# grospy/bitcoincashplus

Measured on AMD Instinct MI355X. Metric: equihash_200_9_solutions_per_sec, higher is better.
Workload: dtype uint32; 1 GPU; model=Equihash(200,9) mainnet PoW solver (BLAKE2b, K=9 collision rounds), global_batch=96, seq_len=2097152, parallelism=dp1 (nonce-space), solvers_in_flight=2, full=False, verified_solutions=0, gpu_cpu_verifier_disagreements=0, rows_dropped_all_nonces=231992, pairs_dropped_all_nonces=346543, candidates_dropped_all_nonces=0

## Files before the change

### csrc/kernels/equihash_solver.hip

```cpp
#include <hip/hip_runtime.h>

#include "crypto/hashes.h"
#include "kernels/blake2b_device.h"
#include "kernels/equihash_pow.h"
#include "kernels/gpu_api.h"
#include "kernels/hip_util.h"

#include <algorithm>
#include <cstdlib>
#include <cstring>
#include <stdexcept>
#include <utility>

#ifndef BCP_EH_XCD_MAP
#define BCP_EH_XCD_MAP 1
#endif
#ifndef BCP_EH_PF_SLICES
#define BCP_EH_PF_SLICES 3
#endif
#ifndef BCP_EH_GEN_HPT
#define BCP_EH_GEN_HPT 2
#endif
#ifndef BCP_EH_GEN_NT
#define BCP_EH_GEN_NT 512
#endif
#ifndef BCP_EH_PRUNE_FROM
#define BCP_EH_PRUNE_FROM 9
#endif
#ifndef BCP_EH_MP_LATE
#define BCP_EH_MP_LATE 1
#endif
#ifndef BCP_EH_MP_LATE_FROM
#define BCP_EH_MP_LATE_FROM 8
#endif
#ifndef BCP_EH_GW
#define BCP_EH_GW 4
#endif
#ifndef BCP_EH_GROUPS_DEFAULT
#define BCP_EH_GROUPS_DEFAULT(batch) ((batch) >= 48 ? (batch) / 24 : 1)
#endif

namespace bcpk {

template <int N_, int K_, int BB_, int CAP_, int NT_, int GENWG_, int NTG_, int MAXCAND_, int CAP4_ = CAP_,
          int CAP3_ = CAP_, int WGCU_ = 1, int GNT_ = 512, int GHPT_ = 2, int CAPF_ = 0, int MPX_ = 0, int GW_ = 0>
struct EhCfg {
    static constexpr int N = N_, K = K_;
    static constexpr int DB = N / (K + 1);
    static constexpr int BB = BB_;
    static constexpr int RB = DB - BB_;
    static constexpr int NB = 1 << BB_;
    static constexpr int NRESTS = 1 << RB;
    static constexpr int CAP = CAP_;
    static constexpr int CAPF = CAPF_ > 0 ? CAPF_ : CAP3_;
    static constexpr int MPX = MPX_;
    static constexpr int cap(int round) {
        return round == K_ ? CAPF : words(round - 1) >= 5 ? CAP_ : words(round - 1) == 4 ? CAP4_ : CAP3_;
    }
    static constexpr int AREA_NF = CAP_ > CAP4_ ? (CAP_ > CAP3_ ? CAP_ : CAP3_) : (CAP4_ > CAP3_ ? CAP4_ : CAP3_);
    static constexpr int AREA = AREA_NF > CAPF ? AREA_NF : CAPF;
    static constexpr int NT = NT_;
    static constexpr int NW = NT_ / 64;
    static constexpr int GW = GW_;
    static constexpr int RNT = NT_ - 64 * GW_;
    static constexpr int WGCU = WGCU_;
    static constexpr int LDS_BUDGET = 160 * 1024 / WGCU_;
    static constexpr int INIT = 1 << (DB + 1);
    static constexpr int GENWG = GENWG_;
    static constexpr int NTG = NTG_;
    static constexpr int GNT = GNT_, GHPT = GHPT_;
    static constexpr int RPW = INIT / GENWG_;
    static constexpr int IPH = 512 / N;
    static constexpr int NBYTES = N / 8;
    static constexpr int MAXCAND = MAXCAND_;
    static constexpr int L = 1 << K;
    static constexpr int bits(int stage) { return N - stage * DB - BB_; }
    static constexpr int words(int stage) { return (bits(stage) + 31) / 32; }
    static constexpr int WMAX = words(0);
    static constexpr int IB = AREA <= 4096 ? 12 : 13;
    static constexpr int DH = 16 - IB;
    static constexpr uint32_t DHM = (1u << DH) - 1;
    static constexpr int DX = 2 * DH;
    static constexpr int DR = BB_ > DX ? BB_ - DX : 0;
    static constexpr uint32_t RMASK = (1u << DR) - 1;
    static constexpr uint32_t IMASK = ((1u << IB) - 1) * 0x10001u;
    static constexpr bool cp(int stage) {
        return stage >= 1 && stage < K && 32 * words(stage) - bits(stage) >= DR;
    }
    static constexpr uint32_t rmask(int stage) { return cp(stage) ? RMASK : 0u; }
    static constexpr int sw(int stage) { return stage == 0 ? words(0) : words(stage) + (cp(stage) ? 1 : 2); }
    static constexpr size_t ROWS = (size_t)NB * AREA;
    static constexpr bool H16 = NB > 512;
    static constexpr int HW = H16 ? NB / 2 : NB;
    static_assert(RPW * GENWG_ == INIT && RPW < 65535, "generation split");
    static_assert(RB > 0 && DB < 32, "digit geometry");
    static_assert(AREA < (1 << IB), "LDS row indices in parent words and signatures");
    static_assert(NT_ % 64 == 0 && NT_ <= 1024 && (NB <= NT_ || NB % NT_ == 0) && NB <= NTG_ && NT_ / 64 <= 64,
                  "workgroup shape");
    static_assert(words(K - 1) == 1, "final round keeps whole rows in one LDS word");
    static_assert(GW_ == 0 || (WGCU_ == 1 && RNT >= 128 && (NB <= RNT || NB % RNT == 0)), "carrying workgroup shape");
};

#ifndef BCP_EH_CAPF
#define BCP_EH_CAPF 6016
#endif
using Cfg200_9 = EhCfg<200, 9, 9, 4416, 1024, 512, 1024, 256, 4864, 5120, 1, BCP_EH_GEN_NT, BCP_EH_GEN_HPT, BCP_EH_CAPF, 0, BCP_EH_GW>;
using Cfg96_5 = EhCfg<96, 5, 7, 1280, 256, 256, 256, 256, 1280, 1280, 1, 512, 2, 0, 1, 1>;
using Cfg48_5 = EhCfg<48, 5, 3, 512, 64, 8, 64, 256>;

constexpr uint32_t NIL = 0xffffffffu;
constexpr uint32_t OOB = 0x80000000u;
typedef uint32_t u2v __attribute__((ext_vector_type(2)));
typedef uint32_t u3v __attribute__((ext_vector_type(3)));
typedef uint32_t u4v __attribute__((ext_vector_type(4)));

template <int CTRL, int ROWMASK = 0xf>
__device__ __forceinline__ uint32_t dpp0(uint32_t x) {
    return (uint32_t)__builtin_amdgcn_update_dpp(0, (int)x, CTRL, ROWMASK, 0xf, false);
}
template <bool MAX> __device__ __forceinline__ uint32_t wave_incl(uint32_t x) {
    auto op = [](uint32_t a, uint32_t b) -> uint32_t { return MAX ? (a > b ? a : b) : a + b; };
    x = op(x, dpp0<0x111>(x));
    x = op(x, dpp0<0x112>(x));
// ... 296 lines not shown
    for (int q = 0; q < G::RPT; ++q) {
        const uint32_t d = rk[q] & 0xffff;
        const uint32_t pos = base[d] + (rk[q] >> 16);
        const uint32_t slot = d * C::AREA + pos;
        const bool ok = pos < OCAP;
        const uint32_t g = g0 + (q / C::IPH) * NTG + tid;
        const uint32_t li = g * C::IPH + (q % C::IPH);
        row_store<W0>(rs, ok ? slot * (SW0 * 4) : OOB, rw[q]);
        __builtin_amdgcn_raw_buffer_store_b32(li, rl, ok ? slot * 4 : OOB, 0, 0);
    }
    }
}

__device__ __forceinline__ uint64_t pack_tri(uint32_t d, uint32_t i, uint32_t j) {
    return ((uint64_t)d << 32) | (j << 16) | i;
}
template <class C> __host__ __device__ __forceinline__ uint32_t cpack(uint32_t d, uint32_t i, uint32_t j) {
    return i | (j << 16) | ((d & C::DHM) << C::IB) | (((d >> C::DH) & C::DHM) << (16 + C::IB));
}
template <class C> __host__ __device__ __forceinline__ uint32_t cunpack_d(uint32_t pw, uint32_t lastword) {
    return ((pw >> C::IB) & C::DHM) | (((pw >> (16 + C::IB)) & C::DHM) << C::DH) | ((lastword & C::RMASK) << C::DX);
}

#define EH_STAMP(k)                                                                                  \
    do {                                                                                             \
        if constexpr (STAMP) {                                                                       \
            if (threadIdx.x == 0) stamps[(size_t)bk * 16 + (k)] = __builtin_amdgcn_s_memtime();        \
        }                                                                                            \
    } while (0)

template <class C> constexpr int un_walk_bend(int cap) { return (cap * 2 + 3) / 4 * 4; }
template <class C> constexpr int un_walk_list(int cap) { return un_walk_bend<C>(cap) + C::NRESTS * 4; }
template <class C> constexpr int round_nt(int stage, bool carry) { return carry && stage < C::K ? C::RNT : C::NT; }
template <class C> constexpr int round_mp(int stage, bool carry = false) {
    const int nt = round_nt<C>(stage, carry);
    return stage == C::K ? 1
                         : (C::AREA_NF + nt - 1) / nt + C::MPX +
                               (C::K == 9 && stage >= BCP_EH_MP_LATE_FROM ? BCP_EH_MP_LATE : 0);
}
template <class C> constexpr int round_un(int stage, bool carry = false) {
    const int cap = C::cap(stage);
    if (stage == C::K) return un_walk_list<C>(cap);
    const int pairs = round_mp<C>(stage, carry) * round_nt<C>(stage, carry) * 4;
    const int walk = un_walk_list<C>(cap) + pairs;
    return walk > pairs ? walk : pairs;
}
template <class C> constexpr int round_lds(int stage, bool prune, bool carry = false) {
    const int WR = C::words(stage - 1);
    const int WI = WR;
    const int cap = C::cap(stage);
    const int pruneb = prune ? cap * 4 + (C::cp(stage - 1) ? 0 : (cap * 2 + 3) / 4 * 4) : 0;
    const int hists = stage == C::K ? 12 : 2 * C::HW * 4 + (C::NB * (C::H16 ? 2 : 4) + 3) / 4 * 4;
    const int gen = carry ? 2 * C::NB * 4 + 16 * 8 : 0;
    return (cap * WI + 3) / 4 * 16 + pruneb + 4 + round_un<C>(stage, carry) + hists +
           (round_nt<C>(stage, carry) / 64 + 1) * 4 + gen;
}
template <class C> constexpr bool round_prunes(int stage, bool carry = false) {
    constexpr int from = C::K == 9 ? BCP_EH_PRUNE_FROM : 2;
    return (stage >= from || stage == C::K) && stage >= 2 && round_lds<C>(stage, true, carry) <= C::LDS_BUDGET;
}

template <class C> struct GenCarry {
    static constexpr int GT = C::GW > 0 ? 64 * C::GW : 64;
    static constexpr int NHASH = (C::INIT + C::IPH - 1) / C::IPH;
    static constexpr int ITERS = (C::K - 1) * C::NB;
    static constexpr int HB = ((NHASH + ITERS - 1) / ITERS + GT - 1) / GT;
    static constexpr int CH = HB * GT;
    static constexpr int RPT = HB * C::IPH;
    static constexpr int BPT = (C::NB + GT - 1) / GT;
    static_assert((long long)CH * ITERS >= NHASH, "the carrying rounds cover every hash");
};
struct EhCarry {
    const EhBaseState* states;
    uint32_t* R0;
    uint32_t* LEAF;
    uint32_t* CTR0;
    int nonces;
};

constexpr int EH_NBAR = 10;
constexpr int EH_SCAN_BARS = 2;
template <int K> __device__ __forceinline__ void eh_bar() {
    static_assert(K >= 1 && K <= EH_NBAR, "barrier outside the bucket iteration's count");
    __syncthreads();
}
#define EH_BAR_SCAN(k) static_assert((k) >= 1 && (k) + EH_SCAN_BARS - 1 <= EH_NBAR, "scan barriers")

template <class C, int STAGE>
__device__ __forceinline__ void eh_carry_gen(const EhCarry& cy, int nbk, uint32_t* ghist, uint32_t* gbase, uint64_t* gr0p) {
    using GC = GenCarry<C>;
// ... 112 lines not shown
        if (act) {
#pragma unroll
            for (int k = 0; k < GC::BPT; ++k) {
                const int b = gtid + k * GT;
                if (b < C::NB) gbase[b] = myb[k];
            }
        }
        eh_bar<9>();
        if (act) {
            const auto rs = buf_rsrc(cy.R0 + (size_t)nonce * C::ROWS * SW0, (uint32_t)(C::ROWS * SW0 * 4));
            const auto rl = buf_rsrc(cy.LEAF + (size_t)nonce * C::ROWS, (uint32_t)(C::ROWS * 4));
#pragma unroll
            for (int q = 0; q < GC::RPT; ++q) {
                const uint32_t d = rk[q] & 0xffff;
                const uint32_t pos = gbase[d < (uint32_t)C::NB ? d : 0] + (rk[q] >> 16);
                const uint32_t slot = d * C::AREA + pos;
                const bool ok = rk[q] != NIL && pos < OCAP;
                const uint32_t li = (g0 + (q / C::IPH) * GT) * C::IPH + (q % C::IPH);
                row_store<W0>(rs, ok ? slot * (SW0 * 4) : OOB, rw[q]);
                __builtin_amdgcn_raw_buffer_store_b32(li, rl, ok ? slot * 4 : OOB, 0, 0);
            }
        }
        if (more) start(bn);
        eh_bar<EH_NBAR>();
        if (!more) break;
        bk = bn;
        ++it;
    }
}

template <class C, int STAGE, bool STAMP, bool CARRY = false>
__global__ __launch_bounds__(C::NT) __attribute__((amdgpu_waves_per_eu(C::WGCU * C::NT / 256)))
void eh_round(const uint32_t* __restrict__ Rin, const uint32_t* __restrict__ CTRin, uint32_t* __restrict__ Rout,
              uint32_t* __restrict__ CTRout, uint32_t* __restrict__ ncand, uint64_t* __restrict__ cand,
              uint64_t* __restrict__ stamps, uint32_t* __restrict__ pdrop, int nbk, EhCarry carry) {
    constexpr int WI = C::words(STAGE - 1);
    constexpr int WO = (STAGE < C::K) ? C::words(STAGE) : 1;
    constexpr int CAP = C::cap(STAGE);
    constexpr bool FINAL = STAGE == C::K;
    constexpr int PDW = 2 * C::K + 2;
    static_assert(!CARRY || (C::GW > 0 && !FINAL && !STAMP), "only plain collision rounds carry generation");
    constexpr bool PRUNE = round_prunes<C>(STAGE, CARRY);
    static_assert(PRUNE == round_prunes<C>(STAGE), "a carrying round prunes like the plain one");
    static_assert(round_lds<C>(STAGE, PRUNE, CARRY) <= 160 * 1024 / C::WGCU, "round LDS budget");
    constexpr int NT = round_nt<C>(STAGE, CARRY);
    static_assert(!CARRY || NT / 64 > 1, "block_exscan runs its two barriers only with more than one wave");
    constexpr int RPL = (CAP + NT - 1) / NT;
    constexpr int MP = round_mp<C>(STAGE, CARRY);
    constexpr int SWI = C::sw(STAGE - 1);
    constexpr int SWO = STAGE < C::K ? C::sw(STAGE) : 1;
    constexpr bool CPI = C::cp(STAGE - 1);
    constexpr uint32_t RMI = C::rmask(STAGE - 1);
    constexpr int SLI = (RPL + BCP_EH_PF_SLICES - 1) / BCP_EH_PF_SLICES;
    constexpr int BPT = (C::NB + NT - 1) / NT;
    constexpr bool FOLD = !FINAL;
    using HT = std::conditional_t<C::H16, uint16_t, uint32_t>;
    __shared__ __attribute__((aligned(16))) uint32_t rows[(CAP * WI + 3) / 4 * 4];
    __shared__ uint32_t psig[PRUNE ? CAP : 1];
    __shared__ uint16_t pdw[PRUNE && !CPI ? CAP : 1];
    __shared__ uint32_t npairs;
    __shared__ __attribute__((aligned(16))) uint8_t un[round_un<C>(STAGE, CARRY)];
    static_assert(FINAL || (sizeof(un) >= (size_t)un_walk_list<C>(CAP) + (size_t)MP * NT * 4),
                  "the union holds sidx, bend and this round's MP * NT pairs");
    __shared__ uint32_t hist_[FINAL ? 1 : C::HW], cur_[FINAL ? 1 : C::HW];
    __shared__ HT base[FINAL ? 1 : C::NB];
    __shared__ uint32_t wsum[NT / 64 + 1];
    __shared__ uint32_t ghist[CARRY ? C::NB : 1], gbase[CARRY ? C::NB : 1];
    __shared__ uint64_t gr0p[CARRY ? 16 : 1];
    uint16_t* sidx = reinterpret_cast<uint16_t*>(un);
    uint32_t* bend = reinterpret_cast<uint32_t*>(un + un_walk_bend<C>(CAP));
    uint32_t* plist = reinterpret_cast<uint32_t*>(un + un_walk_list<C>(CAP));
    uint32_t* spair = FOLD ? plist : reinterpret_cast<uint32_t*>(un);
    const int tid = threadIdx.x;
    const int G = gridDim.x;
    int it = 0;
    int bk = xcd_bucket<C::NB>(blockIdx.x, 0, G, nbk);
    if (bk < 0) return;
    if constexpr (CARRY) {
        if (__builtin_amdgcn_readfirstlane(tid >> 6) >= NT / 64) {
            eh_carry_gen<C, STAGE>(carry, nbk, ghist, gbase, gr0p);
            return;
        }
    }
// ... 42 lines not shown
        dest = (x0 >> (32 - C::DB)) & (C::NB - 1);
        return keep;
    };

    auto opaque_tid = [&]() -> uint32_t {
        uint32_t t;
        asm volatile("v_mov_b32 %0, %1" : "=v"(t) : "v"(tid));
        return t;
    };
    constexpr int LWI = PRUNE ? (CPI ? WI + 1 : WI + 2) : WI;
    uint32_t nr[RPL][LWI];
    uint32_t krank[FOLD ? RPL : 1];
    int pf_bk = bk;
    uint32_t pf_n = 0;
    auto issue = [&](int u0, int u1) {
        const int nonce = pf_bk / C::NB, d = pf_bk % C::NB;
        const auto rs = buf_rsrc(Rin + ((size_t)nonce * C::ROWS + (size_t)d * C::AREA) * SWI, CAP * SWI * 4);
        const uint32_t ot = opaque_tid();
#pragma unroll
        for (int u = 0; u < RPL; ++u) {
            if (u < u0 || u >= u1) continue;
            const uint32_t r = ot + u * NT;
            row_load<LWI>(rs, r < pf_n ? r * (SWI * 4) : OOB, nr[u]);
        }
    };

    uint32_t fill = CTRin[bk];
    uint32_t n = min(fill, (uint32_t)CAP);
    pf_n = n;
    issue(0, RPL);
    if constexpr (!FINAL) {
        const auto rs_out = buf_rsrc(Rout, 0);
        const uint32_t z[SWO] = {};
#pragma unroll
        for (int u = 0; u < MP; ++u) row_store<SWO>(rs_out, OOB + 256 * u, z);
    }
    if constexpr (FOLD) {
        for (int k = tid; k < C::NRESTS; k += NT) bend[k] = 0;
        __syncthreads();
    }
    const int bk1 = xcd_bucket<C::NB>(blockIdx.x, 1, G, nbk);
    uint32_t fill_next = bk1 >= 0 ? CTRin[bk1] : 0u;
    const auto ctr_rs = buf_rsrc(CTRin, (uint32_t)nbk * 4);
    auto fill_of = [&](int b) -> uint32_t {
        return __builtin_amdgcn_raw_buffer_load_b32(ctr_rs, b >= 0 ? (uint32_t)b * 4 : OOB, 0, 0);
    };

    for (;;) {
        const int nonce = bk / C::NB, d = bk % C::NB;
        EH_STAMP(0);
        if (tid == 0 && fill > (uint32_t)CAP) atomicAdd(&pdrop[nonce * PDW + C::K + STAGE], fill - CAP);
        {
            const uint32_t ot = opaque_tid();
#pragma unroll
            for (int u = 0; u < RPL; ++u) {
                const uint32_t r = ot + u * NT;
                if (r < n) {
                    if constexpr (WI % 2 == 0) {
#pragma unroll
                        for (int w = 0; w < WI; w += 2)
                            *reinterpret_cast<u2v*>(&rows[r * WI + w]) = u2v{nr[u][w], nr[u][w + 1]};
                    } else {
#pragma unroll
                        for (int w = 0; w < WI; ++w) rows[r * WI + w] = nr[u][w];
                    }
                    if constexpr (PRUNE) {
                        psig[r] = nr[u][WI];
                        if constexpr (!CPI) pdw[r] = (uint16_t)nr[u][WI + 1];
// ... 103 lines not shown
                    uint32_t dest;
                    if (pair_keep(i, j, dest)) {
                        pv[u] = (j << 16) | i;
                        pd[u] = dest;
                        hinc(hist_, pd[u]);
                    }
                }
            }
            for (int k = tid; k < C::NRESTS; k += NT) bend[k] = 0;
            eh_bar<6>();
            EH_STAMP(4);
            uint32_t myb[BPT];
#pragma unroll
            for (int k = 0; k < BPT; ++k) {
                const int b = tid * BPT + k;
                myb[k] = 0;
                if (b < C::NB) myb[k] = atomicAdd(&CTRout[(size_t)nonce * C::NB + b], hget(hist_, b));
            }
            issue(2 * SLI, RPL);
            uint32_t start = 0;
            uint32_t np;
            EH_BAR_SCAN(7);
            if constexpr (C::H16)
                np = block_exscan<NT, BPT, uint16_t, uint16_t>(reinterpret_cast<const uint16_t*>(hist_),
                                                               reinterpret_cast<uint16_t*>(cur_), C::NB, wsum, &start);
            else
                np = block_exscan<NT, BPT>(hist_, cur_, C::NB, wsum, &start);
#pragma unroll
            for (int u = 0; u < MP; ++u)
                if (pv[u] != NIL) spair[hinc(cur_, pd[u])] = pv[u];
#pragma unroll
            for (int k = 0; k < BPT; ++k) {
                const int b = tid * BPT + k;
                if (b < C::NB) {
                    base[b] = (HT)(myb[k] - start);
                    start += hget(hist_, b);
                }
            }
            eh_bar<9>();
            EH_STAMP(5);
            constexpr uint32_t OCAP = C::cap(STAGE + 1 <= C::K ? STAGE + 1 : C::K);
            constexpr uint32_t RMO = C::rmask(STAGE);
            const auto rs_out = buf_rsrc(Rout + (size_t)nonce * C::ROWS * SWO, (uint32_t)(C::ROWS * SWO * 4));
#pragma unroll
            for (int u = 0; u < MP; ++u) {
                const uint32_t t = tid + u * NT;
                const uint32_t pr = t < np ? spair[t] : 0u;
                const uint32_t i = pr & 0xffff, j = pr >> 16;
                uint32_t x[WI + 1], o[WO];
                lds_row_xor<WI>(rows, i, j, x);
                x[WI - 1] &= ~RMI;
                x[WI] = 0;
                const uint32_t b = (x[0] >> (32 - C::DB)) & (C::NB - 1);
                const uint32_t pos = (HT)(base[b] + t);
                const bool ok = t < np && pos < OCAP;
                const uint32_t slot = b * C::AREA + pos;
#pragma unroll
                for (int w = 0; w < WO; ++w) o[w] = (x[w] << C::DB) | (x[w + 1] >> (32 - C::DB));
                uint32_t ov[SWO] = {};
#pragma unroll
                for (int w = 0; w < WO; ++w) ov[w] = o[w];
                if constexpr (C::cp(STAGE)) {
                    ov[WO - 1] |= (d >> C::DX) & RMO;
                    ov[WO] = cpack<C>(d, i, j);
                } else {
                    ov[WO] = (j << 16) | i;
                    ov[WO + 1] = d;
                }
                row_store<SWO>(rs_out, ok ? slot * (SWO * 4) : OOB, ov);
            }
        }
        eh_bar<EH_NBAR>();
        EH_STAMP(6);
        if (!more) break;
        bk = bn;
        ++it;
        fill = fn;
        n = nn;
    }
}


struct EhStages {
    const uint32_t* r[16];
};
template <class C>
__global__ __launch_bounds__(C::L < 64 ? 64 : C::L) void eh_expand(const uint32_t* __restrict__ LEAF, EhStages st,
                                                                  const uint32_t* __restrict__ ncand,
                                                                  const uint64_t* __restrict__ cand,
                                                                  uint32_t* __restrict__ out_idx,
                                                                  uint32_t* __restrict__ out_valid,
                                                                  uint32_t* __restrict__ nout,
                                                                  uint32_t* __restrict__ out_list) {
    constexpr int L = C::L;
    __shared__ uint32_t buf[2][L];
    __shared__ uint64_t tri[L / 2 > 0 ? L / 2 : 1];
    __shared__ uint32_t dup;
    const uint32_t c = blockIdx.x % C::MAXCAND;
    const uint32_t nonce = blockIdx.x / C::MAXCAND;
    const uint32_t t = threadIdx.x;
    const uint32_t nc = min(ncand[nonce], (uint32_t)C::MAXCAND);
    if (c >= nc) return;
    if (t == 0) {
        tri[0] = cand[(size_t)nonce * C::MAXCAND + c];
        dup = 0;
    }
    int cur = 0;
    for (int s = C::K; s >= 1; --s) {
        __syncthreads();
        const uint32_t cnt = 1u << (C::K - s);
        if (t < 2 * cnt) {
            const uint64_t tr = tri[t >> 1];
            const uint32_t dd = (uint32_t)(tr >> 32);
            const uint32_t r = (t & 1) ? (((uint32_t)tr >> 16) & 0xffff) : ((uint32_t)tr & 0xffff);
            const bool in = dd < (uint32_t)C::NB && r < (uint32_t)C::AREA;
            if (!in) dup = 1;
            buf[cur][t] = in ? dd * C::AREA + r : 0u;
        }
        __syncthreads();
        if (s > 1 && t < 2 * cnt) {
            const uint32_t* q = st.r[s - 1] + ((size_t)nonce * C::ROWS + buf[cur][t]) * C::sw(s - 1) + C::words(s - 1);
            if (C::cp(s - 1))
                tri[t] = ((uint64_t)cunpack_d<C>(q[0], q[-1]) << 32) | (q[0] & C::IMASK);
            else
                tri[t] = ((uint64_t)q[1] << 32) | q[0];
        }
    }
    __syncthreads();
    if (t < (uint32_t)L) buf[cur][t] = LEAF[(size_t)nonce * C::ROWS + buf[cur][t]];
    for (int l = 0; l < C::K; ++l) {
        __syncthreads();
        if (t < (uint32_t)L) {
            const uint32_t w = 1u << l;
            const uint32_t j = t & ~(2 * w - 1);
            const bool swap = buf[cur][j + w] < buf[cur][j];
            const uint32_t pos = t - j;
            const uint32_t np = swap ? (pos < w ? pos + w : pos - w) : pos;
            buf[cur ^ 1][j + np] = buf[cur][t];
        }
        cur ^= 1;
    }
    __syncthreads();
    if (t < (uint32_t)L) out_idx[((size_t)nonce * C::MAXCAND + c) * L + t] = buf[cur][t];
    const int o = cur ^ 1;
    if (t < (uint32_t)L) buf[o][t] = buf[cur][t];
    for (uint32_t k = 2; k <= (uint32_t)L; k <<= 1) {
        for (uint32_t jj = k >> 1; jj > 0; jj >>= 1) {
            __syncthreads();
            if (t < (uint32_t)L) {
                const uint32_t ixj = t ^ jj;
                if (ixj > t) {
                    const uint32_t a = buf[o][t], bb = buf[o][ixj];
                    const bool up = (t & k) == 0;
                    if ((a > bb) == up) {
                        buf[o][t] = bb;
// ... 30 lines not shown
    CBlake2b st = st_in;
    Blake2bState& s = st.MutableState();
    if (s.buflen == 128) {
        s.t[0] += 128;
        if (s.t[0] < 128) s.t[1]++;
        CBlake2b::Compress(s.h, s.buf, s.t[0], s.t[1], false);
        s.buflen = 0;
    }
    if (s.buflen + 4 > 128) throw std::runtime_error("MakeEhBaseState: g would straddle a block boundary");
    if (s.t[1] != 0) throw std::runtime_error("MakeEhBaseState: input too long");
    EhBaseState bs;
    memset(&bs, 0, sizeof(bs));
    memcpy(bs.h, s.h, sizeof(bs.h));
    unsigned char block[128] = {0};
    memcpy(block, s.buf, s.buflen);
    for (int i = 0; i < 16; ++i) memcpy(&bs.m[i], block + 8 * i, 8);
    bs.t0 = s.t[0] + s.buflen + 4;
    bs.g_byte = s.buflen;
    bs.outlen = s.outlen;
    return bs;
}

struct EquihashGpuSolver::Impl {
    unsigned n, k;
    int batch, device;
    hipStream_t stream = nullptr;
    hipEvent_t ev0 = nullptr, ev1 = nullptr;
    hipEvent_t ev_gen = nullptr, ev_rounds = nullptr;
    const Impl* after = nullptr;
    DevBuf<bcpk::EhBaseState> d_states;
    DevBuf<uint32_t> d_ctr, d_leaf, d_ncand, d_idx, d_valid, d_pdrop, d_nout, d_out;
    DevBuf<uint64_t> d_cand;
    DevBuf<uint32_t> d_rst[16];
    HostBuf<bcpk::EhBaseState> h_states;
    HostBuf<uint32_t> h_ncand, h_idx, h_ctr0, h_ctr_all, h_pdrop, h_nout, h_out;
    size_t outq = 0;
    size_t rows = 0, L = 0, maxcand = 0, nb = 0, kstages = 0;
    std::vector<size_t> caps;
    std::vector<size_t> slot_words, row_words;
    uint32_t cp_ib = 0, cp_dh = 0, cp_dhm = 0, cp_dx = 0, cp_rmask = 0, cp_imask = 0;
    std::vector<bool> compact;
    int inflight = 0;
    DevBuf<uint32_t> d_in140, d_powctr, d_win;
    HostBuf<uint32_t> h_powctr, h_win;
    size_t winw = 0;
    const bcpk::EhPowParams* pow = nullptr;
    bool pow_inflight = false;
    bool pow_collect = false;
    EhPowJob pow_job;
    int ncu = 1;
    int groups = 1;
    bool debug = false, stamp_mode = false;
    DevBuf<uint64_t> d_stamps;
    EhGpuStats stats;
    size_t bytes = 0;

    template <class C> void alloc() {
        rows = C::ROWS;
        L = C::L;
        maxcand = C::MAXCAND;
        nb = C::NB;
        caps.clear();
        for (int r = 1; r <= C::K; ++r) caps.push_back(C::cap(r));
        slot_words.clear();
        compact.clear();
        row_words.clear();
        for (int st = 0; st < C::K; ++st) {
            slot_words.push_back(C::sw(st));
            compact.push_back(C::cp(st));
            row_words.push_back(C::words(st));
        }
        kstages = C::K;
        d_states.alloc(batch);
        h_states.alloc(batch);
        static_assert(C::K <= 16, "stage arrays");
        for (int s = 0; s < C::K; ++s) d_rst[s].alloc((size_t)batch * C::ROWS * C::sw(s));
        d_ctr.alloc((size_t)C::K * batch * C::NB);
        d_leaf.alloc((size_t)batch * C::ROWS);
        cp_ib = C::IB, cp_dh = C::DH, cp_dhm = C::DHM, cp_dx = C::DX, cp_rmask = C::RMASK, cp_imask = C::IMASK;
        d_ncand.alloc(batch);
        d_pdrop.alloc((size_t)batch * (2 * C::K + 2));
        h_pdrop.alloc((size_t)batch * (2 * C::K + 2));
        d_cand.alloc((size_t)batch * C::MAXCAND);
        d_idx.alloc((size_t)batch * C::MAXCAND * C::L);
        d_valid.alloc((size_t)batch * C::MAXCAND);
        h_ncand.alloc(batch);
        d_nout.alloc(1);
        h_nout.alloc(1);
        d_out.alloc((size_t)batch * C::MAXCAND * (C::L + 2));
        h_out.alloc((size_t)batch * C::MAXCAND * (C::L + 2));
        outq = std::min<size_t>((size_t)batch * 4 + 16, (size_t)batch * C::MAXCAND);
        h_idx.alloc((size_t)C::MAXCAND * C::L);
        h_ctr0.alloc((size_t)C::K * C::NB);
        h_ctr_all.alloc((size_t)C::K * batch * C::NB);
        d_stamps.alloc((size_t)C::K * batch * C::NB * 16);
        bytes = d_leaf.n * 4 + d_ctr.n * 4 + d_idx.n * 4;
        for (int s = 0; s < C::K; ++s) bytes += d_rst[s].n * 4;
    }

    template <class C, int S, bool ST, bool CY> int round_grid(int nbk) {
        static int per_cu = -1;
        if (per_cu < 0) {
            int occ = 0;
            BCP_HIP_CHECK(hipOccupancyMaxActiveBlocksPerMultiprocessor(&occ, bcpk::eh_round<C, S, ST, CY>, C::NT, 0));
            per_cu = std::max(occ, 1);
        }
        return std::min(nbk, ncu * per_cu);
    }
    template <class C, int S> void launch_round(int noff, int gn, int next) {
        const size_t o = (size_t)noff;
        constexpr size_t PDW = 2 * C::K + 2;
        const uint32_t* rin = d_rst[S - 1].p + o * C::ROWS * C::sw(S - 1);
        uint32_t* rout = S < C::K ? d_rst[S].p + o * C::ROWS * C::sw(S < C::K ? S : 0) : nullptr;
        const uint32_t* cin = d_ctr.p + ((size_t)(S - 1) * batch + o) * C::NB;
        uint32_t* cout = S < C::K ? d_ctr.p + ((size_t)S * batch + o) * C::NB : nullptr;
        uint32_t* nc = d_ncand.p + o;
        uint64_t* cd = d_cand.p + o * C::MAXCAND;
        const int nbk = C::NB * gn;
        bcpk::EhCarry cy{};
        if constexpr (C::GW > 0 && S < C::K) {
            if (next > 0 && !stamp_mode) {
                const size_t p = o + (size_t)gn;
                cy.states = d_states.p + p;
                cy.R0 = d_rst[0].p + p * C::ROWS * C::sw(0);
                cy.LEAF = d_leaf.p + p * C::ROWS;
                cy.CTR0 = d_ctr.p + p * C::NB;
                cy.nonces = next;
                hipLaunchKernelGGL((bcpk::eh_round<C, S, false, true>), dim3(round_grid<C, S, false, true>(nbk)),
                                   dim3(C::NT), 0, stream, rin, cin, rout, cout, nc, cd, nullptr,
                                   d_pdrop.p + o * PDW, nbk, cy);
                ++stats.carry_launches;
                return;
            }
        }
        if (stamp_mode) {
            uint64_t* st = d_stamps.p + ((size_t)(S - 1) * batch + o) * C::NB * 16;
            hipLaunchKernelGGL((bcpk::eh_round<C, S, true>), dim3(round_grid<C, S, true, false>(nbk)), dim3(C::NT), 0,
                               stream, rin, cin, rout, cout, nc, cd, st, d_pdrop.p + o * PDW, nbk, cy);
        } else {
            hipLaunchKernelGGL((bcpk::eh_round<C, S, false>), dim3(round_grid<C, S, false, false>(nbk)), dim3(C::NT), 0,
                               stream, rin, cin, rout, cout, nc, cd, nullptr, d_pdrop.p + o * PDW, nbk, cy);
        }
    }
    template <class C, int... S> void launch_rounds(int noff, int gn, int next, std::integer_sequence<int, S...>) {
        (launch_round<C, S + 1>(noff, gn, next), ...);
    }

    template <class C> void alloc_pow() {
        using P = bcpk::PowCfg<C::N, C::K>;
        if (d_win.n) return;
        winw = P::WINW;
        d_in140.alloc((size_t)batch * 35);
        d_powctr.alloc(2);
        h_powctr.alloc(2);
        d_win.alloc((size_t)batch * C::MAXCAND * P::WINW);
        h_win.alloc((size_t)batch * C::MAXCAND * P::WINW);
    }

    template <class C> void launch(size_t nstates) {
        if (pow) {
            BCP_HIP_CHECK(hipMemsetAsync(d_powctr.p, 0, 2 * sizeof(uint32_t), stream));
            hipLaunchKernelGGL((bcpk::eh_nonce_states<bcpk::PowCfg<C::N, C::K>>), dim3(((int)nstates + 63) / 64), dim3(64),
                               0, stream, *pow, (int)nstates, d_in140.p, d_states.p);
        } else
            BCP_HIP_CHECK(hipMemcpyAsync(d_states.p, h_states.p, nstates * sizeof(bcpk::EhBaseState),
                                         hipMemcpyHostToDevice, stream));
        BCP_HIP_CHECK(hipMemsetAsync(d_ncand.p, 0, batch * sizeof(uint32_t), stream));
        BCP_HIP_CHECK(hipMemsetAsync(d_nout.p, 0, sizeof(uint32_t), stream));
        BCP_HIP_CHECK(hipMemsetAsync(d_pdrop.p, 0, d_pdrop.n * sizeof(uint32_t), stream));
        BCP_HIP_CHECK(hipMemsetAsync(d_ctr.p, 0, d_ctr.n * sizeof(uint32_t), stream));
        if (debug) {
            if (d_leaf.n) BCP_HIP_CHECK(hipMemsetAsync(d_leaf.p, 0xff, d_leaf.n * sizeof(uint32_t), stream));
            for (int s = 0; s < C::K; ++s)
                if (d_rst[s].n) BCP_HIP_CHECK(hipMemsetAsync(d_rst[s].p, 0xff, d_rst[s].n * sizeof(uint32_t), stream));
        }
        BCP_HIP_CHECK(hipEventRecord(ev0, stream));
        bool hdr = true;
        for (size_t i = 0; i < nstates && !pow; ++i) {
            const bcpk::EhBaseState& st = h_states.p[i];
            hdr &= st.g_byte == 12;
            for (int w = 2; w < 16; ++w) hdr &= st.m[w] == 0;
        }
        int gsz = (int)nstates;
        if (C::GW > 0 && hdr && !stamp_mode && groups > 1) {
            gsz = ((int)nstates + groups - 1) / groups;
            if (gsz >= bcpk::NXCD) gsz = (gsz + bcpk::NXCD - 1) / bcpk::NXCD * bcpk::NXCD;
        }
        const int gen_n = std::min(gsz, (int)nstates);
        uint32_t* r0 = d_rst[0].p;
        hipStream_t gs = stream;
        if (after) BCP_HIP_CHECK(hipStreamWaitEvent(gs, after->ev_gen, 0));
        constexpr bool reg = bcpk::GenReg<C, C::GNT, C::GHPT>::OK;
        if constexpr (reg) {
            using GR = bcpk::GenReg<C, C::GNT, C::GHPT>;
            const int items = GR::GWG * gen_n;
            const int grid = items;
            if (hdr)
                hipLaunchKernelGGL((bcpk::eh_gen_reg<C, true, C::GNT, C::GHPT>), dim3(grid), dim3(C::GNT), 0, gs,
                                   d_states.p, r0, d_leaf.p, d_ctr.p, items);
            else
                hipLaunchKernelGGL((bcpk::eh_gen_reg<C, false, C::GNT, C::GHPT>), dim3(grid), dim3(C::GNT), 0, gs,
                                   d_states.p, r0, d_leaf.p, d_ctr.p, items);
        } else if (hdr)
            hipLaunchKernelGGL((bcpk::eh_gen<C, true>), dim3(C::GENWG * gen_n), dim3(C::NTG), 0, gs,
                               d_states.p, r0, d_leaf.p, d_ctr.p);
        else
            hipLaunchKernelGGL((bcpk::eh_gen<C, false>), dim3(C::GENWG * gen_n), dim3(C::NTG), 0, gs,
                               d_states.p, r0, d_leaf.p, d_ctr.p);
        BCP_HIP_CHECK(hipEventRecord(ev_gen, gs));
        if (after) BCP_HIP_CHECK(hipStreamWaitEvent(stream, after->ev_rounds, 0));
        for (int noff = 0; noff < (int)nstates; noff += gsz) {
            const int gn = std::min(gsz, (int)nstates - noff);
            const int next = std::max(0, std::min(gsz, (int)nstates - noff - gsz));
            launch_rounds<C>(noff, gn, next, std::make_integer_sequence<int, C::K>{});
        }
        constexpr int EB = C::L < 64 ? 64 : C::L;
        bcpk::EhStages stages{};
        for (int s = 0; s < C::K; ++s) stages.r[s] = d_rst[s].p;
        hipLaunchKernelGGL((bcpk::eh_expand<C>), dim3(C::MAXCAND * nstates), dim3(EB), 0, stream, d_leaf.p, stages,
                           d_ncand.p, d_cand.p, d_idx.p, d_valid.p, d_nout.p, d_out.p);
        BCP_HIP_CHECK(hipEventRecord(ev_rounds, stream));
        if (pow) {
            using P = bcpk::PowCfg<C::N, C::K>;
            const int grid = (int)std::min<size_t>(C::MAXCAND * nstates, 2048);
            hipLaunchKernelGGL((bcpk::eh_pow_filter<P>), dim3(grid), dim3(64), 0, stream, *pow, (int)nstates, d_in140.p,
                               d_nout.p, d_out.p, (uint32_t)(C::MAXCAND * nstates), d_powctr.p, d_win.p, debug ? 1 : 0);
        }
        BCP_HIP_CHECK(hipGetLastError());
        BCP_HIP_CHECK(hipEventRecord(ev1, stream));
        BCP_HIP_CHECK(
            hipMemcpyAsync(h_ncand.p, d_ncand.p, nstates * sizeof(uint32_t), hipMemcpyDeviceToHost, stream));
        BCP_HIP_CHECK(hipMemcpyAsync(h_pdrop.p, d_pdrop.p, d_pdrop.n * sizeof(uint32_t), hipMemcpyDeviceToHost, stream));
        if (debug) {
            for (int s = 0; s < C::K; ++s)
                BCP_HIP_CHECK(hipMemcpyAsync(h_ctr0.p + (size_t)s * C::NB, d_ctr.p + (size_t)s * batch * C::NB,
                                             C::NB * sizeof(uint32_t), hipMemcpyDeviceToHost, stream));
            BCP_HIP_CHECK(hipMemcpyAsync(h_ctr_all.p, d_ctr.p, d_ctr.n * sizeof(uint32_t), hipMemcpyDeviceToHost, stream));
        }
        BCP_HIP_CHECK(hipMemcpyAsync(h_nout.p, d_nout.p, sizeof(uint32_t), hipMemcpyDeviceToHost, stream));
        if (pow) {
            BCP_HIP_CHECK(hipMemcpyAsync(h_powctr.p, d_powctr.p, 2 * sizeof(uint32_t), hipMemcpyDeviceToHost, stream));
            BCP_HIP_CHECK(hipMemcpyAsync(h_win.p, d_win.p, outq * winw * sizeof(uint32_t), hipMemcpyDeviceToHost, stream));
        } else
            BCP_HIP_CHECK(hipMemcpyAsync(h_out.p, d_out.p, outq * (C::L + 2) * sizeof(uint32_t), hipMemcpyDeviceToHost,
                                         stream));
        if (debug)
            BCP_HIP_CHECK(hipMemcpyAsync(h_idx.p, d_idx.p, C::MAXCAND * C::L * sizeof(uint32_t),
                                         hipMemcpyDeviceToHost, stream));
    }
};

// ... 71 lines not shown
void EquihashGpuSolver::ResetStats() { impl->stats = EhGpuStats(); }

std::vector<uint32_t> EquihashGpuSolver::DebugFills(int nonce) {
    const Impl& m = *impl;
    if (!m.debug || nonce < 0 || nonce >= m.batch) throw std::invalid_argument("DebugFills: debug mode and a nonce of the batch");
    BCP_HIP_CHECK(hipSetDevice(m.device));
    BCP_HIP_CHECK(hipStreamSynchronize(m.stream));
    std::vector<uint32_t> out;
    for (size_t s = 0; s < m.kstages; ++s) {
        const uint32_t* p = m.h_ctr_all.p + (s * m.batch + nonce) * m.nb;
        out.insert(out.end(), p, p + m.nb);
    }
    return out;
}

std::vector<uint64_t> EquihashGpuSolver::DebugDump(int nonce) {
    if (nonce < 0 || nonce >= impl->batch) throw std::invalid_argument("DebugDump: nonce outside the batch");
    BCP_HIP_CHECK(hipSetDevice(impl->device));
    BCP_HIP_CHECK(hipStreamSynchronize(impl->stream));
    const Impl& m = *impl;
    const size_t R = m.rows, K = m.kstages;
    std::vector<uint64_t> out(K * R);
    std::vector<uint32_t> leaf(R);
    BCP_HIP_CHECK(hipMemcpy(leaf.data(), m.d_leaf.p + (size_t)nonce * R, R * 4, hipMemcpyDeviceToHost));
    for (size_t i = 0; i < R; ++i) out[i] = leaf[i];
    auto cunpack_d = [&](uint32_t pw, uint32_t last) {
        return ((pw >> m.cp_ib) & m.cp_dhm) | (((pw >> (16 + m.cp_ib)) & m.cp_dhm) << m.cp_dh) |
               ((last & m.cp_rmask) << m.cp_dx);
    };
    for (size_t s = 1; s < K; ++s) {
        const size_t sw = m.slot_words[s], w = m.row_words[s];
        std::vector<uint32_t> buf(R * sw);
        BCP_HIP_CHECK(hipMemcpy(buf.data(), m.d_rst[s].p + (size_t)nonce * R * sw, R * sw * 4, hipMemcpyDeviceToHost));
        for (size_t i = 0; i < R; ++i) {
            const uint32_t* q = &buf[i * sw + w];
            if (m.compact[s] && q[0] == 0xffffffffu)
                out[s * R + i] = ~0ull;
            else
                out[s * R + i] = m.compact[s] ? ((uint64_t)cunpack_d(q[0], q[-1]) << 32) | (q[0] & m.cp_imask)
                                              : ((uint64_t)q[1] << 32) | q[0];
        }
    }
    return out;
}
size_t EquihashGpuSolver::DeviceBytes() const { return impl->bytes; }

std::vector<uint32_t> EquihashGpuSolver::DebugExpandCorrupt(int mode) {
    BCP_HIP_CHECK(hipSetDevice(impl->device));
    BCP_HIP_CHECK(hipStreamSynchronize(impl->stream));
    Impl& m = *impl;
    uint32_t nc = 0;
    BCP_HIP_CHECK(hipMemcpy(&nc, m.d_ncand.p, 4, hipMemcpyDeviceToHost));
    nc = std::min<uint32_t>(nc, (uint32_t)m.maxcand);
    if (nc == 0) return {};
    uint64_t tri = 0;
    BCP_HIP_CHECK(hipMemcpy(&tri, m.d_cand.p, 8, hipMemcpyDeviceToHost));
    const size_t st = m.kstages - 1;
    const uint32_t d = (uint32_t)(tri >> 32), i = (uint32_t)tri & 0xffff;
    uint32_t* slot = m.d_rst[st].p + ((size_t)d * (m.rows / m.nb) + i) * m.slot_words[st] + m.row_words[st];
    if (mode != 0) {
        if (m.compact[st]) {
            uint32_t w = 0;
            BCP_HIP_CHECK(hipMemcpy(&w, slot, 4, hipMemcpyDeviceToHost));
            w = mode == 1 ? (w | (m.cp_dhm << m.cp_ib) | (m.cp_dhm << (16 + m.cp_ib))) : (w | ((1u << m.cp_ib) - 1));
            BCP_HIP_CHECK(hipMemcpy(slot, &w, 4, hipMemcpyHostToDevice));
        } else {
            uint32_t w[2];
            BCP_HIP_CHECK(hipMemcpy(w, slot, 8, hipMemcpyDeviceToHost));
            if (mode == 1) w[1] = 0xffffu;
            else w[0] = (w[0] & 0xffff0000u) | 0xffffu;
            BCP_HIP_CHECK(hipMemcpy(slot, w, 8, hipMemcpyHostToDevice));
        }
    }
    BCP_HIP_CHECK(hipMemsetAsync(m.d_nout.p, 0, 4, m.stream));
    dispatch_cfg(m.n, m.k, [&](auto c) {
        using C = decltype(c);
        constexpr int EB = C::L < 64 ? 64 : C::L;
        bcpk::EhStages stages{};
        for (int s2 = 0; s2 < C::K; ++s2) stages.r[s2] = m.d_rst[s2].p;
        hipLaunchKernelGGL((bcpk::eh_expand<C>), dim3(C::MAXCAND), dim3(EB), 0, m.stream, m.d_leaf.p, stages,
                           m.d_ncand.p, m.d_cand.p, m.d_idx.p, m.d_valid.p, m.d_nout.p, m.d_out.p);
    });
    BCP_HIP_CHECK(hipGetLastError());
    BCP_HIP_CHECK(hipStreamSynchronize(m.stream));
    std::vector<uint32_t> valid(nc);
    BCP_HIP_CHECK(hipMemcpy(valid.data(), m.d_valid.p, nc * 4, hipMemcpyDeviceToHost));
    return valid;
}

void EquihashGpuSolver::Launch(const std::vector<EhBaseState>& states) {
    if (states.empty() || (int)states.size() > impl->batch) throw std::invalid_argument("bad number of states");
    if (impl->inflight) throw std::runtime_error("EquihashGpuSolver: Collect() the previous launch first");
    BCP_HIP_CHECK(hipSetDevice(impl->device));
    memcpy(impl->h_states.p, states.data(), states.size() * sizeof(EhBaseState));
    dispatch_cfg(impl->n, impl->k, [&](auto c) { impl->launch<decltype(c)>(states.size()); });
    impl->inflight = (int)states.size();
}

void EquihashGpuSolver::Launch(const std::vector<EhBaseState>& states, const EquihashGpuSolver& prev) {
    if (&prev == this) throw std::invalid_argument("EquihashGpuSolver: cannot pipeline behind itself");
    if (prev.impl->device != impl->device) throw std::invalid_argument("EquihashGpuSolver: pipelined solvers on different devices");
    impl->after = prev.impl.get();
    try {
        Launch(states);
    } catch (...) {
        impl->after = nullptr;
        throw;
    }
    impl->after = nullptr;
}

void EquihashGpuSolver::LaunchPow(const EhPowJob& job) {
// ... 198 lines not shown
```

Baseline: 9858 Sol/s.

## Store round parents in side pair/base tables instead of per-row slot words

For middle stages that have enough padding bits and no pruning in the next round, output rows no longer carry the parent index words. Each row keeps only its bucket id in the spare high bits. The pair ordinal is written once per emitted pair into a per-bucket pair table, and per-bucket output bases go into a base table. The expand kernel and the debug readers rebuild parents through these tables. The aim is to shrink slot width and the row store/load traffic in the memory-bound collision rounds, at the cost of extra table writes, extra memory, and indirect lookups during expansion.

```diff
diff --git a/csrc/kernels/equihash_solver.hip b/csrc/kernels/equihash_solver.hip
--- a/csrc/kernels/equihash_solver.hip
+++ b/csrc/kernels/equihash_solver.hip
@@ -36,11 +36,18 @@
 #ifndef BCP_EH_GW
 #define BCP_EH_GW 4
 #endif
+#ifndef BCP_EH_TABLE_PARENTS
+#define BCP_EH_TABLE_PARENTS 1
+#endif
 #ifndef BCP_EH_GROUPS_DEFAULT
 #define BCP_EH_GROUPS_DEFAULT(batch) ((batch) >= 48 ? (batch) / 24 : 1)
 #endif
 
 namespace bcpk {
+
+template <class C> constexpr int round_nt(int stage, bool carry);
+template <class C> constexpr int round_mp(int stage, bool carry = false);
+template <class C> constexpr bool round_prunes(int stage, bool carry = false);
 
 template <int N_, int K_, int BB_, int CAP_, int NT_, int GENWG_, int NTG_, int MAXCAND_, int CAP4_ = CAP_,
           int CAP3_ = CAP_, int WGCU_ = 1, int GNT_ = 512, int GHPT_ = 2, int CAPF_ = 0, int MPX_ = 0, int GW_ = 0>
@@ -87,8 +94,21 @@
     static constexpr bool cp(int stage) {
         return stage >= 1 && stage < K && 32 * words(stage) - bits(stage) >= DR;
     }
-    static constexpr uint32_t rmask(int stage) { return cp(stage) ? RMASK : 0u; }
-    static constexpr int sw(int stage) { return stage == 0 ? words(0) : words(stage) + (cp(stage) ? 1 : 2); }
+    static constexpr int pad(int stage) { return 32 * words(stage) - bits(stage); }
+    static constexpr bool tp(int stage) {
+        return BCP_EH_TABLE_PARENTS && stage >= 1 && stage <= K - 2 && !round_prunes<EhCfg>(stage + 1) &&
+               !round_prunes<EhCfg>(stage + 1, true) && pad(stage) >= BB;
+    }
+    static constexpr int ptab(int stage) {
+        const int a = round_mp<EhCfg>(stage, false) * round_nt<EhCfg>(stage, false);
+        const int b = GW_ > 0 ? round_mp<EhCfg>(stage, true) * round_nt<EhCfg>(stage, true) : 0;
+        return a > b ? a : b;
+    }
+    static constexpr uint32_t tpmask(int stage) { return (1u << (pad(stage) > BB ? BB + 1 : BB)) - 1; }
+    static constexpr uint32_t rmask(int stage) { return tp(stage) ? (uint32_t)NB - 1 : cp(stage) ? RMASK : 0u; }
+    static constexpr int sw(int stage) {
+        return stage == 0 || tp(stage) ? words(stage) : words(stage) + (cp(stage) ? 1 : 2);
+    }
     static constexpr size_t ROWS = (size_t)NB * AREA;
     static constexpr bool H16 = NB > 512;
     static constexpr int HW = H16 ? NB / 2 : NB;
@@ -451,7 +471,7 @@
 template <class C> constexpr int un_walk_bend(int cap) { return (cap * 2 + 3) / 4 * 4; }
 template <class C> constexpr int un_walk_list(int cap) { return un_walk_bend<C>(cap) + C::NRESTS * 4; }
 template <class C> constexpr int round_nt(int stage, bool carry) { return carry && stage < C::K ? C::RNT : C::NT; }
-template <class C> constexpr int round_mp(int stage, bool carry = false) {
+template <class C> constexpr int round_mp(int stage, bool carry) {
     const int nt = round_nt<C>(stage, carry);
     return stage == C::K ? 1
                          : (C::AREA_NF + nt - 1) / nt + C::MPX +
@@ -474,7 +494,7 @@
     return (cap * WI + 3) / 4 * 16 + pruneb + 4 + round_un<C>(stage, carry) + hists +
            (round_nt<C>(stage, carry) / 64 + 1) * 4 + gen;
 }
-template <class C> constexpr bool round_prunes(int stage, bool carry = false) {
+template <class C> constexpr bool round_prunes(int stage, bool carry) {
     constexpr int from = C::K == 9 ? BCP_EH_PRUNE_FROM : 2;
     return (stage >= from || stage == C::K) && stage >= 2 && round_lds<C>(stage, true, carry) <= C::LDS_BUDGET;
 }
@@ -653,8 +673,9 @@
 template <class C, int STAGE, bool STAMP, bool CARRY = false>
 __global__ __launch_bounds__(C::NT) __attribute__((amdgpu_waves_per_eu(C::WGCU * C::NT / 256)))
 void eh_round(const uint32_t* __restrict__ Rin, const uint32_t* __restrict__ CTRin, uint32_t* __restrict__ Rout,
-              uint32_t* __restrict__ CTRout, uint32_t* __restrict__ ncand, uint64_t* __restrict__ cand,
-              uint64_t* __restrict__ stamps, uint32_t* __restrict__ pdrop, int nbk, EhCarry carry) {
+              uint32_t* __restrict__ CTRout, uint32_t* __restrict__ Pout, uint32_t* __restrict__ Bout,
+              uint32_t* __restrict__ ncand, uint64_t* __restrict__ cand, uint64_t* __restrict__ stamps,
+              uint32_t* __restrict__ pdrop, int nbk, EhCarry carry) {
     constexpr int WI = C::words(STAGE - 1);
     constexpr int WO = (STAGE < C::K) ? C::words(STAGE) : 1;
     constexpr int CAP = C::cap(STAGE);
@@ -670,6 +691,10 @@
     constexpr int MP = round_mp<C>(STAGE, CARRY);
     constexpr int SWI = C::sw(STAGE - 1);
     constexpr int SWO = STAGE < C::K ? C::sw(STAGE) : 1;
+    constexpr bool TPO = !FINAL && C::tp(STAGE);
+    constexpr int PTW = TPO ? C::ptab(STAGE) : 1;
+    static_assert(!TPO || PTW >= MP * NT, "the pair table holds every ordinal this round's emit can have (the spair bound)");
+    static_assert(!(PRUNE && C::tp(STAGE - 1)), "a pruning round reads its parents from the slots");
     constexpr bool CPI = C::cp(STAGE - 1);
     constexpr uint32_t RMI = C::rmask(STAGE - 1);
     constexpr int SLI = (RPL + BCP_EH_PF_SLICES - 1) / BCP_EH_PF_SLICES;
@@ -778,8 +803,15 @@
     if constexpr (!FINAL) {
         const auto rs_out = buf_rsrc(Rout, 0);
         const uint32_t z[SWO] = {};
-#pragma unroll
-        for (int u = 0; u < MP; ++u) row_store<SWO>(rs_out, OOB + 256 * u, z);
+        if constexpr (TPO) {
+#pragma unroll
+            for (int k = 0; k < BPT; ++k) __builtin_amdgcn_raw_buffer_store_b32(0u, rs_out, OOB + 256 * MP + 64 * k, 0, 0);
+        }
+#pragma unroll
+        for (int u = 0; u < MP; ++u) {
+            row_store<SWO>(rs_out, OOB + 256 * u, z);
+            if constexpr (TPO) __builtin_amdgcn_raw_buffer_store_b32(0u, rs_out, OOB + 256 * u + 128, 0, 0);
+        }
     }
     if constexpr (FOLD) {
         for (int k = tid; k < C::NRESTS; k += NT) bend[k] = 0;
@@ -949,9 +981,14 @@
 #pragma unroll
             for (int k = 0; k < BPT; ++k) {
                 const int b = tid * BPT + k;
+                const uint32_t rb = myb[k] - start;
                 if (b < C::NB) {
-                    base[b] = (HT)(myb[k] - start);
+                    base[b] = (HT)rb;
                     start += hget(hist_, b);
+                }
+                if constexpr (TPO) {
+                    const auto rs_b = buf_rsrc(Bout + ((size_t)nonce * C::NB + d) * C::NB, C::NB * 4);
+                    __builtin_amdgcn_raw_buffer_store_b32(rb, rs_b, b < C::NB ? (uint32_t)b * 4 : OOB, 0, 0);
                 }
             }
             eh_bar<9>();
@@ -959,6 +996,7 @@
             constexpr uint32_t OCAP = C::cap(STAGE + 1 <= C::K ? STAGE + 1 : C::K);
             constexpr uint32_t RMO = C::rmask(STAGE);
             const auto rs_out = buf_rsrc(Rout + (size_t)nonce * C::ROWS * SWO, (uint32_t)(C::ROWS * SWO * 4));
+            const auto rs_p = buf_rsrc(Pout + (TPO ? ((size_t)nonce * C::NB + d) * PTW : 0), TPO ? PTW * 4 : 0);
 #pragma unroll
             for (int u = 0; u < MP; ++u) {
                 const uint32_t t = tid + u * NT;
@@ -977,7 +1015,9 @@
                 uint32_t ov[SWO] = {};
 #pragma unroll
                 for (int w = 0; w < WO; ++w) ov[w] = o[w];
-                if constexpr (C::cp(STAGE)) {
+                if constexpr (TPO) {
+                    ov[WO - 1] |= (uint32_t)d & RMO;
+                } else if constexpr (C::cp(STAGE)) {
                     ov[WO - 1] |= (d >> C::DX) & RMO;
                     ov[WO] = cpack<C>(d, i, j);
                 } else {
@@ -985,6 +1025,7 @@
                     ov[WO + 1] = d;
                 }
                 row_store<SWO>(rs_out, ok ? slot * (SWO * 4) : OOB, ov);
+                if constexpr (TPO) __builtin_amdgcn_raw_buffer_store_b32(pr, rs_p, t < np ? t * 4 : OOB, 0, 0);
             }
         }
         eh_bar<EH_NBAR>();
@@ -1000,6 +1041,8 @@
 
 struct EhStages {
     const uint32_t* r[16];
+    const uint32_t* p[16];
+    const uint32_t* b[16];
 };
 template <class C>
 __global__ __launch_bounds__(C::L < 64 ? 64 : C::L) void eh_expand(const uint32_t* __restrict__ LEAF, EhStages st,
@@ -1037,7 +1080,15 @@
         __syncthreads();
         if (s > 1 && t < 2 * cnt) {
             const uint32_t* q = st.r[s - 1] + ((size_t)nonce * C::ROWS + buf[cur][t]) * C::sw(s - 1) + C::words(s - 1);
-            if (C::cp(s - 1))
+            if (C::tp(s - 1)) {
+                const uint32_t area = buf[cur][t] / C::AREA, pos = buf[cur][t] % C::AREA;
+                uint32_t d = q[-1] & C::tpmask(s - 1);
+                if (d >= (uint32_t)C::NB) d = 0, dup = 1;
+                const size_t db = (size_t)nonce * C::NB + d;
+                uint32_t o = pos - st.b[s - 1][db * C::NB + area];
+                if (o >= (uint32_t)C::ptab(s - 1)) o = 0, dup = 1;
+                tri[t] = ((uint64_t)d << 32) | st.p[s - 1][db * C::ptab(s - 1) + o];
+            } else if (C::cp(s - 1))
                 tri[t] = ((uint64_t)cunpack_d<C>(q[0], q[-1]) << 32) | (q[0] & C::IMASK);
             else
                 tri[t] = ((uint64_t)q[1] << 32) | q[0];
@@ -1134,6 +1185,10 @@
     DevBuf<uint32_t> d_ctr, d_leaf, d_ncand, d_idx, d_valid, d_pdrop, d_nout, d_out;
     DevBuf<uint64_t> d_cand;
     DevBuf<uint32_t> d_rst[16];
+    DevBuf<uint32_t> d_ptab[16], d_btab[16];
+    std::vector<bool> table;
+    std::vector<size_t> ptab_words;
+    std::vector<uint32_t> tp_mask;
     HostBuf<bcpk::EhBaseState> h_states;
     HostBuf<uint32_t> h_ncand, h_idx, h_ctr0, h_ctr_all, h_pdrop, h_nout, h_out;
     size_t outq = 0;
@@ -1172,11 +1227,24 @@
             compact.push_back(C::cp(st));
             row_words.push_back(C::words(st));
         }
+        table.clear();
+        ptab_words.clear();
+        tp_mask.clear();
+        for (int st = 0; st < C::K; ++st) {
+            table.push_back(C::tp(st));
+            ptab_words.push_back(C::tp(st) ? C::ptab(st) : 0);
+            tp_mask.push_back(C::tp(st) ? C::tpmask(st) : 0u);
+        }
         kstages = C::K;
         d_states.alloc(batch);
         h_states.alloc(batch);
         static_assert(C::K <= 16, "stage arrays");
         for (int s = 0; s < C::K; ++s) d_rst[s].alloc((size_t)batch * C::ROWS * C::sw(s));
+        for (int s = 0; s < C::K; ++s)
+            if (C::tp(s)) {
+                d_ptab[s].alloc((size_t)batch * C::NB * C::ptab(s));
+                d_btab[s].alloc((size_t)batch * C::NB * C::NB);
+            }
         d_ctr.alloc((size_t)C::K * batch * C::NB);
         d_leaf.alloc((size_t)batch * C::ROWS);
         cp_ib = C::IB, cp_dh = C::DH, cp_dhm = C::DHM, cp_dx = C::DX, cp_rmask = C::RMASK, cp_imask = C::IMASK;
@@ -1197,7 +1265,7 @@
         h_ctr_all.alloc((size_t)C::K * batch * C::NB);
         d_stamps.alloc((size_t)C::K * batch * C::NB * 16);
         bytes = d_leaf.n * 4 + d_ctr.n * 4 + d_idx.n * 4;
-        for (int s = 0; s < C::K; ++s) bytes += d_rst[s].n * 4;
+        for (int s = 0; s < C::K; ++s) bytes += (d_rst[s].n + d_ptab[s].n + d_btab[s].n) * 4;
     }
 
     template <class C, int S, bool ST, bool CY> int round_grid(int nbk) {
@@ -1216,6 +1284,9 @@
         uint32_t* rout = S < C::K ? d_rst[S].p + o * C::ROWS * C::sw(S < C::K ? S : 0) : nullptr;
         const uint32_t* cin = d_ctr.p + ((size_t)(S - 1) * batch + o) * C::NB;
         uint32_t* cout = S < C::K ? d_ctr.p + ((size_t)S * batch + o) * C::NB : nullptr;
+        constexpr bool TP = S < C::K && C::tp(S < C::K ? S : 0);
+        uint32_t* pout = TP ? d_ptab[S < C::K ? S : 0].p + o * C::NB * C::ptab(S < C::K ? S : 0) : nullptr;
+        uint32_t* bout = TP ? d_btab[S < C::K ? S : 0].p + o * C::NB * C::NB : nullptr;
         uint32_t* nc = d_ncand.p + o;
         uint64_t* cd = d_cand.p + o * C::MAXCAND;
         const int nbk = C::NB * gn;
@@ -1229,7 +1300,7 @@
                 cy.CTR0 = d_ctr.p + p * C::NB;
                 cy.nonces = next;
                 hipLaunchKernelGGL((bcpk::eh_round<C, S, false, true>), dim3(round_grid<C, S, false, true>(nbk)),
-                                   dim3(C::NT), 0, stream, rin, cin, rout, cout, nc, cd, nullptr,
+                                   dim3(C::NT), 0, stream, rin, cin, rout, cout, pout, bout, nc, cd, nullptr,
                                    d_pdrop.p + o * PDW, nbk, cy);
                 ++stats.carry_launches;
                 return;
@@ -1238,14 +1309,21 @@
         if (stamp_mode) {
             uint64_t* st = d_stamps.p + ((size_t)(S - 1) * batch + o) * C::NB * 16;
             hipLaunchKernelGGL((bcpk::eh_round<C, S, true>), dim3(round_grid<C, S, true, false>(nbk)), dim3(C::NT), 0,
-                               stream, rin, cin, rout, cout, nc, cd, st, d_pdrop.p + o * PDW, nbk, cy);
+                               stream, rin, cin, rout, cout, pout, bout, nc, cd, st, d_pdrop.p + o * PDW, nbk, cy);
         } else {
             hipLaunchKernelGGL((bcpk::eh_round<C, S, false>), dim3(round_grid<C, S, false, false>(nbk)), dim3(C::NT), 0,
-                               stream, rin, cin, rout, cout, nc, cd, nullptr, d_pdrop.p + o * PDW, nbk, cy);
+                               stream, rin, cin, rout, cout, pout, bout, nc, cd, nullptr, d_pdrop.p + o * PDW, nbk,
+                               cy);
         }
     }
     template <class C, int... S> void launch_rounds(int noff, int gn, int next, std::integer_sequence<int, S...>) {
         (launch_round<C, S + 1>(noff, gn, next), ...);
+    }
+
+    template <class C> bcpk::EhStages stage_ptrs() const {
+        bcpk::EhStages st{};
+        for (int s = 0; s < C::K; ++s) st.r[s] = d_rst[s].p, st.p[s] = d_ptab[s].p, st.b[s] = d_btab[s].p;
+        return st;
     }
 
     template <class C> void alloc_pow() {
@@ -1275,6 +1353,10 @@
             if (d_leaf.n) BCP_HIP_CHECK(hipMemsetAsync(d_leaf.p, 0xff, d_leaf.n * sizeof(uint32_t), stream));
             for (int s = 0; s < C::K; ++s)
                 if (d_rst[s].n) BCP_HIP_CHECK(hipMemsetAsync(d_rst[s].p, 0xff, d_rst[s].n * sizeof(uint32_t), stream));
+            for (int s = 0; s < C::K; ++s) {
+                if (d_ptab[s].n) BCP_HIP_CHECK(hipMemsetAsync(d_ptab[s].p, 0xff, d_ptab[s].n * sizeof(uint32_t), stream));
+                if (d_btab[s].n) BCP_HIP_CHECK(hipMemsetAsync(d_btab[s].p, 0xff, d_btab[s].n * sizeof(uint32_t), stream));
+            }
         }
         BCP_HIP_CHECK(hipEventRecord(ev0, stream));
         bool hdr = true;
@@ -1317,8 +1399,7 @@
             launch_rounds<C>(noff, gn, next, std::make_integer_sequence<int, C::K>{});
         }
         constexpr int EB = C::L < 64 ? 64 : C::L;
-        bcpk::EhStages stages{};
-        for (int s = 0; s < C::K; ++s) stages.r[s] = d_rst[s].p;
+        const bcpk::EhStages stages = stage_ptrs<C>();
         hipLaunchKernelGGL((bcpk::eh_expand<C>), dim3(C::MAXCAND * nstates), dim3(EB), 0, stream, d_leaf.p, stages,
                            d_ncand.p, d_cand.p, d_idx.p, d_valid.p, d_nout.p, d_out.p);
         BCP_HIP_CHECK(hipEventRecord(ev_rounds, stream));
@@ -1456,6 +1537,24 @@
         const size_t sw = m.slot_words[s], w = m.row_words[s];
         std::vector<uint32_t> buf(R * sw);
         BCP_HIP_CHECK(hipMemcpy(buf.data(), m.d_rst[s].p + (size_t)nonce * R * sw, R * sw * 4, hipMemcpyDeviceToHost));
+        if (m.table[s]) {
+            const size_t NB = m.nb, area = R / NB, pw = m.ptab_words[s];
+            std::vector<uint32_t> bt(NB * NB), pt(NB * pw);
+            BCP_HIP_CHECK(hipMemcpy(bt.data(), m.d_btab[s].p + (size_t)nonce * NB * NB, bt.size() * 4, hipMemcpyDeviceToHost));
+            BCP_HIP_CHECK(hipMemcpy(pt.data(), m.d_ptab[s].p + (size_t)nonce * NB * pw, pt.size() * 4, hipMemcpyDeviceToHost));
+            for (size_t i = 0; i < R; ++i) {
+                const uint32_t* row = &buf[i * sw];
+                bool unwritten = true;
+                for (size_t x = 0; x < w; ++x) unwritten &= row[x] == 0xffffffffu;
+                const uint32_t d = row[w - 1] & m.tp_mask[s];
+                const uint32_t t = d < NB ? (uint32_t)(i % area) - bt[d * NB + i / area] : 0u;
+                if (unwritten)
+                    out[s * R + i] = ~0ull;
+                else
+                    out[s * R + i] = ((uint64_t)d << 32) | (d < NB && t < pw ? pt[d * pw + t] : 0xffffffffu);
+            }
+            continue;
+        }
         for (size_t i = 0; i < R; ++i) {
             const uint32_t* q = &buf[i * sw + w];
             if (m.compact[s] && q[0] == 0xffffffffu)
@@ -1482,7 +1581,32 @@
     const size_t st = m.kstages - 1;
     const uint32_t d = (uint32_t)(tri >> 32), i = (uint32_t)tri & 0xffff;
     uint32_t* slot = m.d_rst[st].p + ((size_t)d * (m.rows / m.nb) + i) * m.slot_words[st] + m.row_words[st];
-    if (mode != 0) {
+    if (mode == 3 || mode == 4) {
+        if (st < 2 || !m.table[st - 1] || m.tp_mask[st - 1] < m.nb)
+            throw std::invalid_argument("DebugExpandCorrupt: modes 3 and 4 need table parents with spare padding in stage K-2");
+        uint32_t w[2] = {0, 0};
+        BCP_HIP_CHECK(hipMemcpy(w, slot, m.compact[st] ? 4 : 8, hipMemcpyDeviceToHost));
+        uint32_t last = 0;
+        if (m.compact[st]) BCP_HIP_CHECK(hipMemcpy(&last, slot - 1, 4, hipMemcpyDeviceToHost));
+        const uint32_t d1 = m.compact[st] ? ((w[0] >> m.cp_ib) & m.cp_dhm) | (((w[0] >> (16 + m.cp_ib)) & m.cp_dhm) << m.cp_dh) |
+                                                ((last & m.cp_rmask) << m.cp_dx)
+                                          : w[1];
+        const uint32_t i1 = (m.compact[st] ? w[0] & m.cp_imask : w[0]) & 0xffff;
+        const size_t area = m.rows / m.nb;
+        if (d1 >= m.nb || i1 >= area) throw std::runtime_error("DebugExpandCorrupt: the first candidate's parent is out of range");
+        uint32_t* lw = m.d_rst[st - 1].p + ((size_t)d1 * area + i1) * m.slot_words[st - 1] + m.row_words[st - 1] - 1;
+        uint32_t x = 0;
+        BCP_HIP_CHECK(hipMemcpy(&x, lw, 4, hipMemcpyDeviceToHost));
+        if (mode == 3) {
+            x |= (uint32_t)m.nb;
+            BCP_HIP_CHECK(hipMemcpy(lw, &x, 4, hipMemcpyHostToDevice));
+        } else {
+            const uint32_t d2 = x & m.tp_mask[st - 1];
+            if (d2 >= m.nb) throw std::runtime_error("DebugExpandCorrupt: the parent row's bucket is out of range");
+            const uint32_t rb = i1 - (uint32_t)m.ptab_words[st - 1];
+            BCP_HIP_CHECK(hipMemcpy(m.d_btab[st - 1].p + (size_t)d2 * m.nb + d1, &rb, 4, hipMemcpyHostToDevice));
+        }
+    } else if (mode != 0) {
         if (m.compact[st]) {
             uint32_t w = 0;
             BCP_HIP_CHECK(hipMemcpy(&w, slot, 4, hipMemcpyDeviceToHost));
@@ -1500,8 +1624,7 @@
     dispatch_cfg(m.n, m.k, [&](auto c) {
         using C = decltype(c);
         constexpr int EB = C::L < 64 ? 64 : C::L;
-        bcpk::EhStages stages{};
-        for (int s2 = 0; s2 < C::K; ++s2) stages.r[s2] = m.d_rst[s2].p;
+        const bcpk::EhStages stages = m.stage_ptrs<C>();
         hipLaunchKernelGGL((bcpk::eh_expand<C>), dim3(C::MAXCAND), dim3(EB), 0, m.stream, m.d_leaf.p, stages,
                            m.d_ncand.p, m.d_cand.p, m.d_idx.p, m.d_valid.p, m.d_nout.p, m.d_out.p);
     });
```

Result: faster. 10050 Sol/s (median of 6 runs) (+1.9%).
